# LiMeng95/MultiPoseNet.pytorch

Measured on AMD Instinct MI355X. Metric: images/sec (train fwd+bwd) ResNet101 480x480 bs=32/GPU, higher is better.
Workload: dtype bf16; 1 GPU; R101 full posenet (keypoint+detection) train step: fwd + MSE/focal losses + bwd + Adam, 480x480, 32 images/GPU, bf16 MFMA / fp32 accumulate / fp32 master weights; global_batch=32, parallelism=dp1, loss_log=asynchronous (set_lazy_log), launch=recorded launch list re-issued per step (replay.py), 88 replays, optimizer_update=Adam in one launch after backward

## Files before the change

### include/mpn.h

```cpp
#ifndef MPN_H_
#define MPN_H_
#include <stdint.h>

#ifdef __cplusplus
extern "C" {
#endif

#define MPN_F32 0
#define MPN_BF16 1
#define MPN_F16 2

#define MPN_E_BADARG (-2)
#define MPN_E_UNSUPPORTED (-3)

typedef struct MpnConvParams {
    const void* x;
    const void* w;
    void* y;
    const float* bias;
    const float* scale;
    const void* res;
    const uint8_t* res_mask;
    float* stats;
    int64_t x_sB, x_sH, x_sW;
// ... 81 lines not shown
int mpn_conv_wgrad_reduce(const MpnWgradParams* p, void* stream);
int mpn_conv_wgrad_kernel_id(const MpnWgradParams* p);

int mpn_reduce_partials(const float* ws, int chunks, int64_t n, float* dst, int accumulate, void* stream);

int mpn_cast_f32_to_bf16(const float* src, void* dst, int64_t n, void* stream);
int mpn_cast_f32(const float* src, void* dst, int64_t n, int dtype, void* stream);
int mpn_weight_transpose(const float* w, void* wt, int Cout, int RS, int Cin, int Cout_pad,
                         int dtype, void* stream);
int mpn_weight_transpose_batched(const float* arena, void* dst, const int64_t* table, int nlayers, int64_t nblocks,
                                 int dtype, void* stream);
int mpn_weight_pad_k(const float* w, void* dst, int Cout, int K, int Kpad, int dtype, void* stream);
int mpn_stem_pack_weight(const float* w, void* packed, int Cout, int dtype, void* stream);
int mpn_stem_unpack_wgrad(const float* dpacked, float* dw, int Cout, void* stream);
int mpn_stem_pack_image(const float* img, int64_t sB, int64_t sC, int64_t sH, int64_t sW, void* dst,
                        int B, int H, int W, int dtype, void* stream);

int mpn_bn_finalize_train(const float* stats, int tiles, int C, int64_t count, const float* gamma,
                          const float* beta, float* running_mean, float* running_var, float momentum,
                          float eps, float* mean, float* invstd, float* scale, float* shift, void* stream);
int mpn_bn_finalize_eval(int C, const float* gamma, const float* beta, const float* running_mean,
                         const float* running_var, float eps, float* mean, float* invstd,
                         float* scale, float* shift, void* stream);
int mpn_bn_act_forward(const void* y, const void* res, void* z, const float* scale, const float* shift,
                       int64_t P, int C, int Cs, int relu, int dtype, uint8_t* mask, void* stream);
int mpn_bn_bwd_reduce(const void* dz, const void* z, const void* y, const float* mean, const float* invstd,
                      const float* mask_scale, const float* mask_shift, float* partial, int chunks, int64_t P, int C, int Cs, int relu, int dtype, void* stream);
int mpn_bn_bwd_finalize(const float* partial, int chunks, int C, int64_t count, const float* gamma, const float* mean,
                        const float* invstd, int train, float* dgamma, float* dbeta, float* coef, void* stream);
int mpn_bn_bwd_apply(const void* dz, const void* z, const void* y, const float* k1, const float* k2, const float* k3,
                     const float* mask_scale, const float* mask_shift, void* dy, void* dres, int dres_accumulate, int64_t P, int C, int Cs, int relu, int dtype,
                     const uint8_t* mask, void* stream);
int mpn_bn_bwd_chunks(int64_t P, int Cs, int dtype);

int mpn_maxpool3x3s2_forward(const void* x, void* y, uint8_t* idx, int B, int H, int W, int Cs,
                             int Ho, int Wo, int dtype, void* stream);
int mpn_maxpool3x3s2_backward(const void* dy, const uint8_t* idx, void* dx, int B, int H, int W, int Cs,
                              int Ho, int Wo, int dtype, void* stream);
int mpn_upsample_nearest_backward(const void* dfine, void* dcoarse, int B, int Hf, int Wf, int Hc, int Wc,
                                  int Cs, int accumulate, int dtype, void* stream);
int mpn_upsample_nearest_slice(const void* src, void* dst, int B, int Hs, int Ws, int Cs_src,
                               int Ho, int Wo, int Cs_dst, int c_off, int dtype, void* stream);
int mpn_upsample_nearest_slice_backward(const void* ddst, void* dsrc, int B, int Hs, int Ws, int Cs_src,
                                        int Ho, int Wo, int Cs_dst, int c_off, int dtype, void* stream);
int mpn_export_f32(const void* src, int src_dtype, float* dst, int B, int Hs, int Ws, int Cs, int C,
                   int Ho, int Wo, int64_t dst_sB, int64_t dst_sP, void* stream);
int mpn_import_grad(const float* ddst, int64_t ddst_sB, int64_t ddst_sP, void* dsrc, int dst_dtype,
                    int B, int Hs, int Ws, int Cs, int C, int Ho, int Wo, void* stream);
int mpn_nchw_to_nhwc_f32(const float* src, int64_t sB, int64_t sC, int64_t sH, int64_t sW, float* dst,
                         int B, int C, int H, int W, void* stream);
int mpn_det_pack(const void* src, int src_dtype, float* dst, int B, int64_t HW, int Cs, int C, int64_t dst_sB, void* stream);
int mpn_det_unpack(const float* ddst, void* dsrc, int dst_dtype, int B, int64_t HW, int Cs, int C, int64_t dst_sB, void* stream);
int mpn_relu_forward(const void* x, void* y, int64_t n, int dtype, void* stream);
int mpn_relu_backward(const void* dz, const void* z, void* dx, int64_t n, int accumulate, int dtype, void* stream);
int mpn_add_inplace(void* dst, const void* src, int64_t n, int dtype, void* stream);
int mpn_channel_sum(const void* dy, int dy_dtype, int64_t P, int C, int Cs, float* partial, int chunks, void* stream);
int mpn_channel_sum_chunks(int64_t P, int Cs, int dtype);
int mpn_colsum_rows(const void* dy, int dy_dtype, int64_t P, int C, int Cs, float* db, void* stream);

int mpn_mse_heatmap_forward(const float* const* preds, const int64_t* pred_sP, const float* gt, const float* wgt,
                            int64_t npix, float* partial, int chunks, float* out, void* stream);
int mpn_mse_heatmap_backward(const float* const* preds, float* const* dpreds, const int64_t* pred_sP,
                             const int64_t* dpred_sP, const int32_t* pred_C, const float* gt, const float* wgt,
                             int64_t npix, const float* gscale, void* stream);
int mpn_mse_chunks(int64_t npix);
int mpn_mse_train_blocks(int B, int H, int W);
// ... 104 lines not shown
```

### multiposenet/pytorch_amd/_lib.py

```python
import ctypes
import os
import subprocess

import torch

_HERE = os.path.dirname(os.path.abspath(__file__))
LIB_PATH = os.path.join(_HERE, "libmpn_hip.so")
CSRC = os.path.join(_HERE, "csrc")

F32, BF16, F16 = 0, 1, 2


class MpnError(RuntimeError):
    pass


class ConvParams(ctypes.Structure):
    _fields_ = [
        ("x", ctypes.c_void_p), ("w", ctypes.c_void_p), ("y", ctypes.c_void_p),
        ("bias", ctypes.c_void_p), ("scale", ctypes.c_void_p), ("res", ctypes.c_void_p), ("res_mask", ctypes.c_void_p),
        ("stats", ctypes.c_void_p),
        ("x_sB", ctypes.c_int64), ("x_sH", ctypes.c_int64), ("x_sW", ctypes.c_int64),
        ("y_sB", ctypes.c_int64), ("y_sP", ctypes.c_int64),
        ("res_sB", ctypes.c_int64), ("res_sP", ctypes.c_int64),
# ... 42 lines not shown
    "mpn_resize": (_i, [_vp, _i64, _i64, _i64, _i, _i, _i, _vp, _i, _i, _i, ctypes.c_double, ctypes.c_double, _vp]),
    "mpn_prn_build_maps": (_i, [_vp, _vp, _vp, _vp, _i, _i, _i, ctypes.c_double, _vp, _vp, _vp, _vp, _vp]),
    "mpn_prn_scores": (_i, [_vp, _vp, _i, _i, _i, _i, _vp, _vp, _vp]),
    "mpn_prn_scores_compact": (_i, [_vp, _vp, _i, _i, _i, _i, _i, _vp, _vp, _vp, _vp, _vp, _vp]),
    "mpn_prn_match_host": (_i, [_i, _vp, _vp, _vp, _vp, _vp, _vp, _vp, _i, _vp, _i, _i, _vp, _vp]),
    "mpn_conv_stats_tiles": (_i, [_PC]),
    "mpn_conv_tile_rows": (_i, [_PC]),
    "mpn_conv_shared_tile": (_i, [_PC]),
    "mpn_conv_forward": (_i, [_PC, _vp]),
    "mpn_debug_wgrad_prof": (_i, [_vp]),
    "mpn_debug_igemm_prof": (_i, [_vp]),
    "mpn_conv_wgrad_chunks": (_i, [_PW]),
    "mpn_conv_wgrad_seg_plan": (_i, [_PW]),
    "mpn_conv_wgrad": (_i, [_PW, _vp]),
    "mpn_conv_wgrad_partials": (_i, [_PW, _vp]),
    "mpn_conv_wgrad_reduce": (_i, [_PW, _vp]),
    "mpn_conv_wgrad_kernel_id": (_i, [_PW]),
    "mpn_reduce_partials": (_i, [_vp, _i, _i64, _vp, _i, _vp]),
    "mpn_cast_f32_to_bf16": (_i, [_vp, _vp, _i64, _vp]),
    "mpn_cast_f32": (_i, [_vp, _vp, _i64, _i, _vp]),
    "mpn_weight_transpose": (_i, [_vp, _vp, _i, _i, _i, _i, _i, _vp]),
    "mpn_weight_transpose_batched": (_i, [_vp, _vp, _vp, _i, _i64, _i, _vp]),
    "mpn_weight_pad_k": (_i, [_vp, _vp, _i, _i, _i, _i, _vp]),
    "mpn_stem_pack_weight": (_i, [_vp, _vp, _i, _i, _vp]),
    "mpn_stem_unpack_wgrad": (_i, [_vp, _vp, _i, _vp]),
    "mpn_stem_pack_image": (_i, [_vp, _i64, _i64, _i64, _i64, _vp, _i, _i, _i, _i, _vp]),
    "mpn_bn_finalize_train": (_i, [_vp, _i, _i, _i64, _vp, _vp, _vp, _vp, _f, _f, _vp, _vp, _vp, _vp, _vp]),
    "mpn_bn_finalize_eval": (_i, [_i, _vp, _vp, _vp, _vp, _f, _vp, _vp, _vp, _vp, _vp]),
    "mpn_bn_act_forward": (_i, [_vp, _vp, _vp, _vp, _vp, _i64, _i, _i, _i, _i, _vp, _vp]),
    "mpn_bn_bwd_reduce": (_i, [_vp, _vp, _vp, _vp, _vp, _vp, _vp, _vp, _i, _i64, _i, _i, _i, _i, _vp]),
    "mpn_bn_bwd_finalize": (_i, [_vp, _i, _i, _i64, _vp, _vp, _vp, _i, _vp, _vp, _vp, _vp]),
    "mpn_bn_bwd_apply": (_i, [_vp, _vp, _vp, _vp, _vp, _vp, _vp, _vp, _vp, _vp, _i, _i64, _i, _i, _i, _i, _vp, _vp]),
    "mpn_bn_bwd_chunks": (_i, [_i64, _i, _i]),
    "mpn_maxpool3x3s2_forward": (_i, [_vp, _vp, _vp, _i, _i, _i, _i, _i, _i, _i, _vp]),
    "mpn_maxpool3x3s2_backward": (_i, [_vp, _vp, _vp, _i, _i, _i, _i, _i, _i, _i, _vp]),
    "mpn_upsample_nearest_backward": (_i, [_vp, _vp, _i, _i, _i, _i, _i, _i, _i, _i, _vp]),
    "mpn_upsample_nearest_slice": (_i, [_vp, _vp, _i, _i, _i, _i, _i, _i, _i, _i, _i, _vp]),
    "mpn_upsample_nearest_slice_backward": (_i, [_vp, _vp, _i, _i, _i, _i, _i, _i, _i, _i, _i, _vp]),
    "mpn_export_f32": (_i, [_vp, _i, _vp, _i, _i, _i, _i, _i, _i, _i, _i64, _i64, _vp]),
    "mpn_import_grad": (_i, [_vp, _i64, _i64, _vp, _i, _i, _i, _i, _i, _i, _i, _i, _vp]),
    "mpn_nchw_to_nhwc_f32": (_i, [_vp, _i64, _i64, _i64, _i64, _vp, _i, _i, _i, _i, _vp]),
    "mpn_det_pack": (_i, [_vp, _i, _vp, _i, _i64, _i, _i, _i64, _vp]),
    "mpn_det_unpack": (_i, [_vp, _vp, _i, _i, _i64, _i, _i, _i64, _vp]),
    "mpn_relu_forward": (_i, [_vp, _vp, _i64, _i, _vp]),
    "mpn_relu_backward": (_i, [_vp, _vp, _vp, _i64, _i, _i, _vp]),
    "mpn_add_inplace": (_i, [_vp, _vp, _i64, _i, _vp]),
    "mpn_channel_sum": (_i, [_vp, _i, _i64, _i, _i, _vp, _i, _vp]),
    "mpn_colsum_rows": (_i, [_vp, _i, _i64, _i, _i, _vp, _vp]),
    "mpn_channel_sum_chunks": (_i, [_i64, _i, _i]),
    "mpn_mse_chunks": (_i, [_i64]),
    "mpn_mse_heatmap_forward": (_i, [_vp, _vp, _vp, _vp, _i64, _vp, _i, _vp, _vp]),
    "mpn_mse_heatmap_backward": (_i, [_vp, _vp, _vp, _vp, _vp, _vp, _vp, _i64, _vp, _vp]),
    "mpn_mse_train_blocks": (_i, [_i, _i, _i]),
    "mpn_mse_heatmap_train": (_i, [_vp, _vp, _vp, _i, _vp, _vp, _i64, _i64, _i64, _i, _i, _i, _vp, _vp, _i, _vp, _vp]),
    "mpn_focal_blocks": (_i, [_i]),
    "mpn_focal_forward": (_i, [_vp, _vp, _vp, _vp, _i, _i, _i, _vp, _vp, _vp, _vp]),
    "mpn_focal_backward": (_i, [_vp, _vp, _vp, _vp, _i, _i, _i, _vp, _vp, _vp, _vp, _vp]),
    "mpn_focal_mc_blocks": (_i, [_i]),
    "mpn_focal_forward_mc": (_i, [_vp, _vp, _vp, _vp, _i, _i, _i, _i, _vp, _vp, _vp, _vp, _vp]),
    "mpn_focal_backward_mc": (_i, [_vp, _vp, _vp, _vp, _i, _i, _i, _i, _vp, _vp, _vp, _vp, _vp]),
    "mpn_class_max": (_i, [_vp, _i, _i, _i, _vp, _vp, _vp]),
    "mpn_sigmoid_forward": (_i, [_vp, _vp, _i64, _vp]),
    "mpn_gather_dets": (_i, [_vp, _vp, _i, _vp, _vp, _vp]),
    "mpn_sigmoid_backward": (_i, [_vp, _vp, _vp, _i64, _vp]),
    "mpn_add_softmax_rows": (_i, [_vp, _i64, _vp, _vp, _i, _i, _i, _vp]),
    "mpn_softmax_rows_backward": (_i, [_vp, _vp, _vp, _i64, _vp, _i, _i, _vp]),
# ... 113 lines not shown
```

### multiposenet/pytorch_amd/csrc/bn.hip

```cpp
#include "common.h"
#include <stdlib.h>

namespace {

template <typename T> struct Geo {
    static constexpr int V = Vec16<T>::N;
    int G, GB, lanes, g, pl, c0;
    __device__ __forceinline__ Geo(int Cs) {
        G = Cs / V;
        GB = G < 256 ? G : 256;
        lanes = 256 / GB;
        g = blockIdx.y * GB + (threadIdx.x % GB);
        pl = threadIdx.x / GB;
        c0 = g * V;
    }
};

template <int V>
__device__ __forceinline__ void load_coef(const float* __restrict__ p, int c0, int C, float (&out)[V], float fill) {
#pragma unroll
    for (int k = 0; k < V; k += 4) {
        if (p != nullptr && c0 + k + 3 < C) {
            const float4 t = *reinterpret_cast<const float4*>(p + c0 + k);
            out[k] = t.x; out[k + 1] = t.y; out[k + 2] = t.z; out[k + 3] = t.w;
// ... 87 lines not shown
                                                     const float* __restrict__ scale, const float* __restrict__ shift,
                                                     long P, int C, int Cs, int relu, int iters, unsigned char* __restrict__ mask) {
    constexpr int V = Vec16<T>::N;
    const Geo<T> q(Cs);
    float sc[V], sf[V];
    load_coef<V>(scale, q.c0, C, sc, 0.f);
    load_coef<V>(shift, q.c0, C, sf, 0.f);
    const long p0 = (long)blockIdx.x * q.lanes * iters + q.pl;
    for (int it = 0; it < iters; ++it) {
        const long p = p0 + (long)it * q.lanes;
        if (p >= P) break;
        const long off = p * Cs + q.c0;
        Vec16<T> a; a.load(y + off);
        Vec16<T> r;
        if (res) r.load(res + off);
#pragma unroll
        for (int k = 0; k < V; ++k) {
            float x = a.v[k] * sc[k] + sf[k];
            if (res) x += r.v[k];
            if (relu) x = fmaxf(x, 0.f);
            a.v[k] = (q.c0 + k < C) ? x : 0.f;
        }
        a.store(z + off);
        if (mask) {
            unsigned bits = 0;
#pragma unroll
            for (int k = 0; k < V; ++k) bits |= (Elem<T>::round(a.v[k]) > 0.f ? 1u : 0u) << k;
            mask[p * q.G + q.g] = (unsigned char)bits;
        }
    }
}

template <typename T>
__global__ void __launch_bounds__(256) bn_bwd_reduce_kernel(const T* __restrict__ dz, const T* __restrict__ z, const T* __restrict__ y,
                                                            const float* __restrict__ mean, const float* __restrict__ invstd,
                                                            const float* __restrict__ mscale, const float* __restrict__ mshift,
                                                            float* __restrict__ partial, long P, int C, int Cs, int relu, int chunk_pix) {
    constexpr int V = Vec16<T>::N;
    __shared__ float sh[256][2 * V + 1];
    const Geo<T> q(Cs);
    const long p_begin = (long)blockIdx.x * chunk_pix;
    long p_end = p_begin + chunk_pix; if (p_end > P) p_end = P;
    float s1[V], s2[V], mu[V], is[V], sc[V], sf[V];
    load_coef<V>(mean, q.c0, C, mu, 0.f);
    load_coef<V>(invstd, q.c0, C, is, 0.f);
    const bool remask = relu && z == nullptr;
    if (remask) { load_coef<V>(mscale, q.c0, C, sc, 0.f); load_coef<V>(mshift, q.c0, C, sf, 0.f); }
#pragma unroll
    for (int k = 0; k < V; ++k) { s1[k] = 0.f; s2[k] = 0.f; }
    for (long p = p_begin + q.pl; p < p_end; p += q.lanes) {
        const long off = p * Cs + q.c0;
        Vec16<T> d, o, x;
        d.load(dz + off); x.load(y + off);
        if (relu && !remask) o.load(z + off);
#pragma unroll
        for (int k = 0; k < V; ++k) {
            float gk = d.v[k];
            if (remask) o.v[k] = x.v[k] * sc[k] + sf[k];
            if (relu && !(o.v[k] > 0.f)) gk = 0.f;
            s1[k] += gk;
            s2[k] += gk * ((x.v[k] - mu[k]) * is[k]);
        }
    }
#pragma unroll
    for (int k = 0; k < V; ++k) { sh[threadIdx.x][k] = s1[k]; sh[threadIdx.x][V + k] = s2[k]; }
    __syncthreads();
    if (q.pl == 0) {
        for (int l = 1; l < q.lanes; ++l) {
#pragma unroll
            for (int k = 0; k < V; ++k) {
                s1[k] += sh[threadIdx.x + l * q.GB][k];
                s2[k] += sh[threadIdx.x + l * q.GB][V + k];
            }
        }
#pragma unroll
        for (int k = 0; k < V; ++k) {
            const int c = q.c0 + k;
            if (c < C) *reinterpret_cast<float2*>(partial + ((long)blockIdx.x * C + c) * 2) = make_float2(s1[k], s2[k]);
        }
    }
}

__global__ void bn_bwd_finalize_kernel(const float* __restrict__ partial, int chunks, int C, double count,
                                       const float* __restrict__ gamma, const float* __restrict__ mean, const float* __restrict__ invstd,
                                       int train, float* __restrict__ dgamma, float* __restrict__ dbeta, float* __restrict__ coef) {
    __shared__ double sh[2][4][4];
    const int cl = threadIdx.x & 3, sl = threadIdx.x >> 2;
    const int c = blockIdx.x * 4 + cl;
    double s1 = 0.0, s2 = 0.0;
    const bool fin = sl == 0 && c < C;
    const float is = fin ? invstd[c] : 0.f, gm = (fin && gamma) ? gamma[c] : 1.f, mu = fin ? mean[c] : 0.f;
    const float db0 = (fin && dbeta) ? dbeta[c] : 0.f, dg0 = (fin && dgamma) ? dgamma[c] : 0.f;
    if (c < C) reduce_slices(partial, chunks, C, c, sl, s1, s2);
#pragma unroll
    for (int m = 4; m < 64; m <<= 1) { s1 += __shfl_xor(s1, m); s2 += __shfl_xor(s2, m); }
    const int lane = threadIdx.x & 63, wave = threadIdx.x >> 6;
    if (lane < 4) { sh[0][wave][cl] = s1; sh[1][wave][cl] = s2; }
    __syncthreads();
    if (sl == 0 && c < C) {
        s1 = (sh[0][0][cl] + sh[0][1][cl]) + (sh[0][2][cl] + sh[0][3][cl]);
        s2 = (sh[1][0][cl] + sh[1][1][cl]) + (sh[1][2][cl] + sh[1][3][cl]);
        if (dbeta) dbeta[c] = db0 + (float)s1;
        if (dgamma) dgamma[c] = dg0 + (float)s2;
        if (coef) {
            const float a = (float)(s1 / count), b = (float)(s2 / count);
            coef[c] = gm * is;
            coef[C + c] = train ? -gm * is * is * b : 0.f;
            coef[2 * C + c] = train ? gm * is * (mu * is * b - a) : 0.f;
        }
    }
}

template <typename T>
__global__ void __launch_bounds__(256) bn_bwd_apply_kernel(const T* __restrict__ dz, const T* __restrict__ z, const T* __restrict__ y,
                                                           const float* __restrict__ k1p, const float* __restrict__ k2p,
                                                           const float* __restrict__ k3p, const float* __restrict__ mscale,
                                                           const float* __restrict__ mshift, T* __restrict__ dy, T* __restrict__ dres,
                                                           int dres_acc, long P, int C, int Cs, int relu, int iters,
                                                           const unsigned char* __restrict__ mask) {
    constexpr int V = Vec16<T>::N;
    const Geo<T> q(Cs);
    float k1[V], k2[V], k3[V];
    load_coef<V>(k1p, q.c0, C, k1, 0.f);
    load_coef<V>(k2p, q.c0, C, k2, 0.f);
    load_coef<V>(k3p, q.c0, C, k3, 0.f);
    const bool bits = relu && mask != nullptr;
    const bool remask = relu && !bits && z == nullptr;
    float sc[V], sf[V];
    if (remask) { load_coef<V>(mscale, q.c0, C, sc, 0.f); load_coef<V>(mshift, q.c0, C, sf, 0.f); }
    const bool need_y = ((dy != nullptr) && (k2p != nullptr)) || remask;
    const long p0 = (long)blockIdx.x * q.lanes * iters + q.pl;
    for (int it = 0; it < iters; ++it) {
        const long p = p0 + (long)it * q.lanes;
        if (p >= P) break;
        const long off = p * Cs + q.c0;
        Vec16<T> d, o, x, out, r;
        d.load(dz + off);
        if (need_y) x.load(y + off);
        if (relu && !remask && !bits) o.load(z + off);
        unsigned mb = 0;
        if (bits) mb = mask[p * q.G + q.g];
        if (dres && dres_acc) r.load(dres + off);
#pragma unroll
        for (int k = 0; k < V; ++k) {
            float gk = d.v[k];
            if (remask) o.v[k] = x.v[k] * sc[k] + sf[k];
            if (bits) o.v[k] = ((mb >> k) & 1u) ? 1.f : 0.f;
            if (relu && !(o.v[k] > 0.f)) gk = 0.f;
            const bool live = q.c0 + k < C;
            out.v[k] = live ? (k1[k] * gk + (k2p ? k2[k] * x.v[k] : 0.f) + k3[k]) : 0.f;
            if (dres) r.v[k] = (dres_acc ? r.v[k] : 0.f) + (live ? gk : 0.f);
        }
        if (dy) out.store(dy + off);
        if (dres) r.store(dres + off);
    }
}

inline int geo_lanes(int Cs, int V) { const int G = Cs / V; return 256 / (G < 256 ? G : 256); }
inline int geo_yblocks(int Cs, int V) { const int G = Cs / V; return G <= 256 ? 1 : G / 256; }
inline bool geo_ok(int Cs, int V) { const int G = Cs / V; return Cs % V == 0 && G > 0 && (G & (G - 1)) == 0; }

inline int pick_iters(long P, int lanes) {
    static const long blocks = mpn_tune("MPN_BN_BLOCKS", 8192);
    long it = P / ((long)lanes * blocks);
    if (it < 1) it = 1;
    if (it > 32) it = 32;
    return (int)it;
}
inline int reduce_chunk(long P, int lanes) {
    long c = P / 512;
    const long lo = (long)lanes * 4, hi = 4096;
    if (c < lo) c = lo;
    if (c > hi) c = hi;
    return (int)((c + lanes - 1) / lanes * lanes);
}

}

extern "C" int mpn_bn_finalize_train(const float* stats, int tiles, int C, int64_t count, const float* gamma,
                                     const float* beta, float* running_mean, float* running_var, float momentum,
                                     float eps, float* mean, float* invstd, float* scale, float* shift, void* stream) {
    MPN_CHECK_ARG(stats && tiles > 0 && C > 0 && count > 0 && mean && invstd && scale && shift);
    hipLaunchKernelGGL(bn_finalize_train_kernel, dim3((C + 3) / 4), dim3(256), 0, (hipStream_t)stream, stats, tiles, C,
                       (double)count, gamma, beta, running_mean, running_var, momentum, eps, mean, invstd, scale, shift);
    return mpn_launch_status();
}

extern "C" int mpn_bn_finalize_eval(int C, const float* gamma, const float* beta, const float* running_mean,
                                    const float* running_var, float eps, float* mean, float* invstd,
                                    float* scale, float* shift, void* stream) {
// ... 31 lines not shown
    const int chunk = reduce_chunk(P, geo_lanes(Cs, V));
    MPN_CHECK_ARG(chunks == (int)((P + chunk - 1) / chunk));
    dim3 grid((unsigned)chunks, (unsigned)geo_yblocks(Cs, V));
    MPN_DISPATCH_T(dtype, hipLaunchKernelGGL((bn_bwd_reduce_kernel<T>), grid, dim3(256), 0, (hipStream_t)stream, (const T*)dz, (const T*)z,
                           (const T*)y, mean, invstd, mask_scale, mask_shift, partial, (long)P, C, Cs, relu, chunk));
    return mpn_launch_status();
}

extern "C" int mpn_bn_bwd_finalize(const float* partial, int chunks, int C, int64_t count, const float* gamma, const float* mean,
                                   const float* invstd, int train, float* dgamma, float* dbeta, float* coef, void* stream) {
    MPN_CHECK_ARG(partial && chunks > 0 && C > 0 && count > 0);
    MPN_CHECK_ARG(!coef || (mean && invstd));
    hipLaunchKernelGGL(bn_bwd_finalize_kernel, dim3((C + 3) / 4), dim3(256), 0, (hipStream_t)stream, partial, chunks, C,
                       (double)count, gamma, mean, invstd, train, dgamma, dbeta, coef);
    return mpn_launch_status();
}

extern "C" int mpn_bn_bwd_apply(const void* dz, const void* z, const void* y, const float* k1, const float* k2, const float* k3,
                                const float* mask_scale, const float* mask_shift, void* dy, void* dres, int dres_accumulate, int64_t P, int C, int Cs, int relu, int dtype,
                                const uint8_t* mask, void* stream) {
    MPN_CHECK_ARG(dz && (dy || dres) && P > 0 && C > 0 && Cs >= C);
    MPN_CHECK_ARG(!dy || k1);
    MPN_CHECK_ARG(!(dy && k2) || y);
    MPN_CHECK_ARG(!relu || z || mask || (mask_scale && mask_shift && y));
    const int V = dtype == MPN_F32 ? 4 : 8;
    MPN_CHECK_ARG(geo_ok(Cs, V) && C % 4 == 0);
    const int lanes = geo_lanes(Cs, V), iters = pick_iters(P, lanes);
    dim3 grid((unsigned)((P + (long)lanes * iters - 1) / ((long)lanes * iters)), (unsigned)geo_yblocks(Cs, V));
    MPN_DISPATCH_T(dtype, hipLaunchKernelGGL((bn_bwd_apply_kernel<T>), grid, dim3(256), 0, (hipStream_t)stream, (const T*)dz, (const T*)z,
                           (const T*)y, k1, k2, k3, mask_scale, mask_shift, (T*)dy, (T*)dres, dres_accumulate, (long)P, C, Cs, relu, iters,
                           (const unsigned char*)mask));
    return mpn_launch_status();
}
```

### multiposenet/pytorch_amd/engine.py

```python
import ctypes
import os

import torch

from . import ops
from ._lib import MpnError, call, gpu_op
from .ops import Act, round_up


class Ctx(object):

    def __init__(self, train):
        self.train = train
        self.tape = []
        self.grads = {}
        self.keep = []
        self.out_grads = {}
        self.wt = {}
        self.wt_buf = None
        self.uses = {}
        self.bn_train_ran = False
        self.side_keep = []
        self.side_pending = []
        self.wt_ready = None
# ... 24 lines not shown


def num_classes(cm):
    cout = cm.output.weight.shape[0]
    if cout % 9 != 0 or cout == 0 or getattr(cm, "num_anchors", 9) != 9:
        raise MpnError("classificationModel: the output convolution has %d channels; the detector needs 9 anchors x K classes" % cout)
    return cout // 9


def _geom(layer):
    w = layer.weight
    if w.dim() == 2:
        return w.shape[0], w.shape[1], 1, 1, 1, 0
    return w.shape[0], w.shape[1], w.shape[2], w.shape[3], layer.stride[0], layer.padding[0]


class Engine(object):
    def __init__(self, model):
        self.m = model
        self._drop_calls = 0
        self._side = None
        self._wt_plan_cache = None
        self.overlap_wgrad = os.environ.get("MPN_SIDE_STREAM", "1") != "0"
        self.fork_every = max(1, int(os.environ.get("MPN_SIDE_FORK_EVERY", "1")))
        self.pyramid_towers = os.environ.get("MPN_PYRAMID_TOWERS", "1") != "0"
        self.fuse_bn_stats = os.environ.get("MPN_BN_FUSED_STATS", "1") != "0"
        self.fold_bn = os.environ.get("MPN_FOLD_BN", "1") != "0"
        self.fuse_bn_finalize = os.environ.get("MPN_BN_FUSED_FINALIZE", "1") != "0"
        self.det_pyramid_side = int(os.environ.get("MPN_DET_PYRAMID_SIDE", "2"))
        self.bn_mask_bits = os.environ.get("MPN_BN_MASK_BITS", "1") != "0"
        self.defer_shortcut_grad = os.environ.get("MPN_DEFER_SHORTCUT_GRAD", "1") != "0"
        self.virtual_concat = os.environ.get("MPN_VIRTUAL_CONCAT", "1") != "0"
        self.conv2_classes = os.environ.get("MPN_CONV2_CLASSES", "1") != "0"

    def side_stream(self, device):
        if not self.overlap_wgrad or device.type != "cuda":
            return None
        if self._side is None:
            self._side = torch.cuda.Stream(device=device)
        return self._side

    def _on_side(self, ctx, device, keep, fn, torch_ops=False):
        side = self.side_stream(device)
        if side is None:
            fn()
            return
        ctx.side_keep.append(keep)
        ctx.side_pending.append((fn, torch_ops))
        if len(ctx.side_pending) >= self.fork_every:
            self.flush_side(ctx, device)

    def flush_side(self, ctx, device):
        if not ctx.side_pending:
            return
        side = self.side_stream(device)
        pending, ctx.side_pending = ctx.side_pending, []
        ev = torch.cuda.Event()
        gpu_op(ev.record, torch.cuda.current_stream(device))
        gpu_op(side.wait_event, ev)
        for fn, torch_ops in pending:
            if torch_ops:
                with torch.cuda.stream(side):
                    fn()
                continue
            ops.push_stream(side)
            try:
# ... 645 lines not shown
            img = img.float()
        packed = torch.empty((B, Hp, Wp, 4), dtype=self.cdt, device=img.device)
        call("mpn_stem_pack_image", ops.ptr(img), img.stride(0), img.stride(1), img.stride(2), img.stride(3), ops.ptr(packed),
             B, H, W, ops.dtype_code(self.cdt), ops.stream_ptr())
        xa = Act(packed, 4)
        w = f.conv1.weight
        wp = torch.empty((64, 7, 32), dtype=self.cdt, device=img.device)
        call("mpn_stem_pack_weight", ops.ptr(self.m._arena.data_seg(w)), ops.ptr(wp), 64, ops.dtype_code(self.cdt), ops.stream_ptr())
        Ho, Wo = ops.conv_out_hw(H, W, 7, 7, 2, 3)
        geom = (Hp, Wp, Hp * Wp * 4, Wp * 4, 4)
        bn_train = f.bn1.training
        if self.fold_bn and not ctx.train and not bn_train:
            bst = ops.bn_finalize_eval(f.bn1.weight.data, f.bn1.bias.data, f.bn1.running_mean, f.bn1.running_var, f.bn1.eps)
            z, _ = ops.conv_forward(xa, wp, 64, 7, 1, 2, 0, cin=32, x_geom=geom, out_hw=(Ho, Wo), scale=bst.scale, bias=bst.shift, act=1)
            return self.maxpool(ctx, z)
        y, st = ops.conv_forward(xa, wp, 64, 7, 1, 2, 0, cin=32, x_geom=geom, out_hw=(Ho, Wo), want_stats=bn_train,
                                 bn_fin=self._bn_fin(f.bn1) if bn_train else None)
        if ctx.train and w.requires_grad:
            y.needs_grad = True
            self._note_use(ctx, w)

            def bwd():
                dy = ctx.pop_grad(y)
                if dy is not None:
                    dwp = torch.empty((64, 7, 32), dtype=torch.float32, device=img.device)

                    def stem_wgrad():
                        call("mpn_fill_f32", ops.ptr(dwp), 0.0, dwp.numel(), ops.stream_ptr())
                        ops.conv_wgrad(xa, dy, dwp, 64, 7, 1, 2, 0, cin=32, x_geom=geom)
                        call("mpn_stem_unpack_wgrad", ops.ptr(dwp), ops.ptr(self.m._arena.grad_seg(w)), 64, ops.stream_ptr())
                    self._on_side(ctx, dy.t.device, (xa, dy, dwp), stem_wgrad)
                self._grad_done(ctx, w)
            ctx.tape.append(bwd)
        z = self.bn(ctx, y, st, f.bn1, True)
        return self.maxpool(ctx, z)

    def conv_bn(self, ctx, x, conv, bn, relu, res=None):
        if self.fold_bn and not ctx.train and not bn.training:
            st = ops.bn_finalize_eval(bn.weight.data, bn.bias.data, bn.running_mean, bn.running_var, bn.eps)
            O, I, R, S, stride, pad = _geom(conv)
            act = (3 if res is not None else 1) if relu else 0
            y, _ = ops.conv_forward(x, self.w_fwd(conv), O, R, S, stride, pad, scale=st.scale, bias=st.shift, act=act,
                                    res=res, res_mode=1 if res is not None else 0)
            return y
        y, s = self.conv(ctx, x, conv, stats=bn.training, bn=bn)
        return self.bn(ctx, y, s, bn, relu, res=res)

    def bottleneck(self, ctx, x, blk):
        z1 = self.conv_bn(ctx, x, blk.conv1, blk.bn1, True)
        z2 = self.conv_bn(ctx, z1, blk.conv2, blk.bn2, True)
        sc = self.conv_bn(ctx, x, blk.downsample[0], blk.downsample[1], False) if len(blk.downsample) > 0 else x
        return self.conv_bn(ctx, z2, blk.conv3, blk.bn3, True, res=sc)

    def backbone(self, ctx, img):
        f = self.m.fpn
        c = self.stem(ctx, img)
        feats = []
        for layer in (f.layer1, f.layer2, f.layer3, f.layer4):
            for blk in layer:
                c = self.bottleneck(ctx, c, blk)
            feats.append(c)
        return feats

    def det_pyramid(self, ctx, c3, c4, c5):
        f = self.m.fpn

        def coarse(h):
            h["p6"], _ = self.conv(ctx, c5, f.conv6)
# ... 167 lines not shown
```

### multiposenet/pytorch_amd/ops.py

```python
import ctypes
import os

import torch

from . import _lib
from ._lib import BF16, F16, F32, ConvParams, WgradParams, call


def round_up(v, m):
    return (v + m - 1) // m * m


def dtype_code(dt):
    if dt == torch.float32:
        return F32
    if dt == torch.bfloat16:
        return BF16
    if dt == torch.float16:
        return F16
    raise _lib.MpnError("unsupported dtype %s" % dt)


_STREAM_OVERRIDE = []

# ... 717 lines not shown
                 chunks, P, C, Cs, 1 if relu else 0, dc, stream_ptr())
        coef = torch.empty((3, C), dtype=torch.float32, device=dev) if train else None
        call("mpn_bn_bwd_finalize", ptr(part), chunks, C, P, ptr(gamma), ptr(st.mean), ptr(st.invstd), 1 if train else 0,
             ptr(dgamma), ptr(dbeta), ptr(coef), stream_ptr())
        if train:
            k1, k2, k3 = coef[0], coef[1], coef[2]
    dy = None
    if want_dy or dres is not None:
        if want_dy:
            dy = Act(torch.empty_like(y.t), C)
        bits = z.mask if (relu and not remask) else None
        call("mpn_bn_bwd_apply", ptr(dz.t), ptr(z.t) if (relu and not remask and bits is None) else None, ptr(y.t), ptr(k1), ptr(k2), ptr(k3),
             ptr(st.scale) if remask else None, ptr(st.shift) if remask else None,
             ptr(dy.t) if dy is not None else None, ptr(dres.t) if dres is not None else None,
             1 if dres_acc else 0, P, C, Cs, 1 if relu else 0, dc, ptr(bits), stream_ptr())
    return dy


def maxpool_forward(x, needs_grad=False):
    Ho, Wo = (x.H + 2 - 3) // 2 + 1, (x.W + 2 - 3) // 2 + 1
    y = Act(torch.empty((x.B, Ho, Wo, x.Cs), dtype=x.t.dtype, device=x.t.device), x.C, needs_grad)
    idx = torch.empty((x.B, Ho, Wo, x.Cs), dtype=torch.uint8, device=x.t.device) if needs_grad else None
    call("mpn_maxpool3x3s2_forward", ptr(x.t), ptr(y.t), ptr(idx), x.B, x.H, x.W, x.Cs, Ho, Wo, dtype_code(x.t.dtype), stream_ptr())
    return y, idx


def maxpool_backward(dy, idx, x_like):
    dx = Act(torch.empty_like(x_like.t), x_like.C)
    call("mpn_maxpool3x3s2_backward", ptr(dy.t), ptr(idx), ptr(dx.t), x_like.B, x_like.H, x_like.W, x_like.Cs, dy.H, dy.W,
         dtype_code(dy.t.dtype), stream_ptr())
    return dx


def upsample_backward(dfine, dcoarse, accumulate):
    call("mpn_upsample_nearest_backward", ptr(dfine.t), ptr(dcoarse.t), dfine.B, dfine.H, dfine.W, dcoarse.H, dcoarse.W,
         dfine.Cs, 1 if accumulate else 0, dtype_code(dfine.t.dtype), stream_ptr())


def upsample_slice(src, dst, c_off):
    call("mpn_upsample_nearest_slice", ptr(src.t), ptr(dst.t), src.B, src.H, src.W, src.Cs, dst.H, dst.W, dst.Cs, c_off,
         dtype_code(src.t.dtype), stream_ptr())


def upsample_slice_backward(ddst, dsrc, c_off):
    call("mpn_upsample_nearest_slice_backward", ptr(ddst.t), ptr(dsrc.t), dsrc.B, dsrc.H, dsrc.W, dsrc.Cs, ddst.H, ddst.W,
         ddst.Cs, c_off, dtype_code(dsrc.t.dtype), stream_ptr())


def export_f32(src, C, Ho, Wo):
    out = torch.empty((src.B, Ho, Wo, C), dtype=torch.float32, device=src.t.device)
    call("mpn_export_f32", ptr(src.t), dtype_code(src.t.dtype), ptr(out), src.B, src.H, src.W, src.Cs, C, Ho, Wo,
         Ho * Wo * C, C, stream_ptr())
    return out.permute(0, 3, 1, 2)


def import_grad(g_nchw, like, dtype):
    B, C, Ho, Wo = g_nchw.shape
    g = g_nchw.permute(0, 2, 3, 1)
    if g.stride(3) != 1 or g.stride(1) != Wo * g.stride(2):
        g = g.contiguous()
    d = Act(torch.empty((like.B, like.H, like.W, like.Cs), dtype=dtype, device=like.t.device), like.C)
    call("mpn_import_grad", ptr(g), g.stride(0), g.stride(2), ptr(d.t), dtype_code(dtype), like.B, like.H, like.W, like.Cs,
         like.C, Ho, Wo, stream_ptr())
    return d


# ... 163 lines not shown
```

### multiposenet/pytorch_amd/replay.py

```python
import itertools
import math
import os
from collections import OrderedDict

import ctypes

import torch

from . import _lib, ops
from .engine import Ctx
from .network import losses

_epoch = itertools.count(1 << 20)


class _Entry(object):
    __slots__ = ("tape", "pool", "img", "gts", "logv", "names", "keep", "sig", "loss")


class ReplayedTrainStep(object):
    def __init__(self, model, optimizer, eager_steps=1, fused_mse=None, max_entries=None, anno_bucket=8, max_grad_norm=None):
        self.model = model
        self.opt = optimizer
        self.max_grad_norm = None if max_grad_norm is None or math.isinf(max_grad_norm) else float(max_grad_norm)
# ... 77 lines not shown
        return self.bucket_mode == "1" or self.model._reducer is not None

    def _local_schedule(self):
        from .ddp import GradReducer
        ar = self.model._arena
        sc = getattr(self, "_local", None)
        if sc is None or sc.arena is not ar:
            sc = self._local = GradReducer(ar, local=True, bucket_mb=float(os.environ.get("MPN_BUCKET_MB", "32")))
        return sc

    def _ones(self, dev):
        t = getattr(self, "_ones_t", None)
        if t is None or t.device != dev:
            t = self._ones_t = torch.ones(2, dtype=torch.float32, device=dev)
        return t

    @staticmethod
    def _log_names(want_kp, want_det, clip=False):
        names = []
        if want_kp:
            kn = losses.build_names()
            names += [(kn[j * 2], j) for j in range(5)] + [("max_ht", 6), ("min_ht", 7)]
        if want_det:
            names += [("total_loss", 8), ("classification_loss", 9), ("regression_loss", 10)]
        if clip:
            names.append(("max_grad", 12))
        return names

    def _state_sig(self):
        m = self.model
        ar = m._arena
        return (id(ar), id(ar.grad_flat), tuple(p.requires_grad for p in ar.params), tuple(b.training for b in m._bns),
                m.compute_dtype, id(m._reducer), m._engine.overlap_wgrad, m._engine.fork_every, id(self.opt._m), self.bucketed_update,
                m._engine.conv2_classes, m._engine.virtual_concat, self._clip_sig())

    def _clip_sig(self):
        if self.max_grad_norm is None:
            return None
        return tuple(p.grad is not None for p in self.model._arena.params)

    def __call__(self, inputs, gts):
        (img, subnet), = inputs
        gts = list(gts)
        if gts[0] != subnet:
            raise ValueError("inputs and gts name different subnets (%r vs %r)" % (subnet, gts[0]))
        tensors = gts[1:]
        if subnet not in ("keypoint_subnet", "detection_subnet", "train_both"):
            if self.max_grad_norm is not None:
                raise ValueError("recorded train step: %r is not recorded and train_step does not clip; clip it on the eager path "
                                 "(training.trainer._Stepper does)" % (subnet,))
            from .training.batch_processor import train_step
            return train_step(self.model, self.opt, inputs, gts)
        ops.check_device(img)
        img = self._as_f32(img, "image batch")
        tensors = [self._as_f32(g, "target %d" % i) for i, g in enumerate(tensors)]
        if subnet in ("detection_subnet", "train_both") and self.anno_bucket > 1:
            ai = 2 if subnet == "train_both" else 0
            if ai < len(tensors) and tensors[ai].dim() == 3:
                tensors[ai] = self._bucket_annotations(tensors[ai])
        key = (subnet, tuple(img.shape), img.dtype, tuple((tuple(t.shape), t.dtype) for t in tensors))
        ent = self._entries.get(key)
        if ent is not None and ent.sig != self._state_sig():
            ent = None
            self._drop(key)
        if ent is not None:
            self._entries.move_to_end(key)
        if ent is None:
# ... 99 lines not shown
```

Before: 894.1 images/sec.

## Fuse stem BN+ReLU with 3x3 maxpool forward and backward

Adds a kernel that applies the stem's BN scale/shift and ReLU while computing the 3x3 stride-2 maxpool and argmax indices, so the full-resolution activated tensor is never written. The backward pass feeds pooled gradients and indices straight into the BN backward reduce and apply kernels, which rebuild the unpooled gradient on the fly. This removes the maxpool backward kernel and the full-resolution z and dz round trips. In exchange each pixel does extra index gathers, and the work is duplicated across the reduce and apply passes. The path is on by default and can be disabled with an environment flag.

```diff
diff --git a/include/mpn.h b/include/mpn.h
--- a/include/mpn.h
+++ b/include/mpn.h
@@ -137,6 +137,14 @@
                      const float* mask_scale, const float* mask_shift, void* dy, void* dres, int dres_accumulate, int64_t P, int C, int Cs, int relu, int dtype,
                      const uint8_t* mask, void* stream);
 int mpn_bn_bwd_chunks(int64_t P, int Cs, int dtype);
+int mpn_bn_act_maxpool_forward(const void* y, void* out, uint8_t* idx, const float* scale, const float* shift,
+                               int B, int H, int W, int Ho, int Wo, int C, int Cs, int dtype, void* stream);
+int mpn_bn_bwd_reduce_pooled(const void* dp, const uint8_t* idx, const void* y, const float* mean, const float* invstd,
+                             const float* mask_scale, const float* mask_shift, float* partial, int chunks,
+                             int B, int H, int W, int Ho, int Wo, int C, int Cs, int dtype, void* stream);
+int mpn_bn_bwd_apply_pooled(const void* dp, const uint8_t* idx, const void* y, const float* k1, const float* k2, const float* k3,
+                            const float* mask_scale, const float* mask_shift, void* dy,
+                            int B, int H, int W, int Ho, int Wo, int C, int Cs, int dtype, void* stream);
 
 int mpn_maxpool3x3s2_forward(const void* x, void* y, uint8_t* idx, int B, int H, int W, int Cs,
                              int Ho, int Wo, int dtype, void* stream);
diff --git a/multiposenet/pytorch_amd/_lib.py b/multiposenet/pytorch_amd/_lib.py
--- a/multiposenet/pytorch_amd/_lib.py
+++ b/multiposenet/pytorch_amd/_lib.py
@@ -98,6 +98,9 @@
     "mpn_bn_bwd_finalize": (_i, [_vp, _i, _i, _i64, _vp, _vp, _vp, _i, _vp, _vp, _vp, _vp]),
     "mpn_bn_bwd_apply": (_i, [_vp, _vp, _vp, _vp, _vp, _vp, _vp, _vp, _vp, _vp, _i, _i64, _i, _i, _i, _i, _vp, _vp]),
     "mpn_bn_bwd_chunks": (_i, [_i64, _i, _i]),
+    "mpn_bn_act_maxpool_forward": (_i, [_vp] * 5 + [_i] * 8 + [_vp]),
+    "mpn_bn_bwd_reduce_pooled": (_i, [_vp] * 8 + [_i] * 9 + [_vp]),
+    "mpn_bn_bwd_apply_pooled": (_i, [_vp] * 9 + [_i] * 8 + [_vp]),
     "mpn_maxpool3x3s2_forward": (_i, [_vp, _vp, _vp, _i, _i, _i, _i, _i, _i, _i, _vp]),
     "mpn_maxpool3x3s2_backward": (_i, [_vp, _vp, _vp, _i, _i, _i, _i, _i, _i, _i, _vp]),
     "mpn_upsample_nearest_backward": (_i, [_vp, _vp, _i, _i, _i, _i, _i, _i, _i, _i, _vp]),
diff --git a/multiposenet/pytorch_amd/csrc/bn.hip b/multiposenet/pytorch_amd/csrc/bn.hip
--- a/multiposenet/pytorch_amd/csrc/bn.hip
+++ b/multiposenet/pytorch_amd/csrc/bn.hip
@@ -143,14 +143,120 @@
 }
 
 template <typename T>
-__global__ void __launch_bounds__(256) bn_bwd_reduce_kernel(const T* __restrict__ dz, const T* __restrict__ z, const T* __restrict__ y,
-                                                            const float* __restrict__ mean, const float* __restrict__ invstd,
-                                                            const float* __restrict__ mscale, const float* __restrict__ mshift,
-                                                            float* __restrict__ partial, long P, int C, int Cs, int relu, int chunk_pix) {
+__global__ void __launch_bounds__(256) bn_act_maxpool_kernel(const T* __restrict__ y, T* __restrict__ out, unsigned char* __restrict__ idx,
+                                                             const float* __restrict__ scale, const float* __restrict__ shift,
+                                                             int B, int H, int W, int Ho, int Wo, int C, int Cs, int iters) {
     constexpr int V = Vec16<T>::N;
-    __shared__ float sh[256][2 * V + 1];
     const Geo<T> q(Cs);
-    const long p_begin = (long)blockIdx.x * chunk_pix;
+    float sc[V], sf[V];
+    load_coef<V>(scale, q.c0, C, sc, 0.f);
+    load_coef<V>(shift, q.c0, C, sf, 0.f);
+    const int Po = B * Ho * Wo;
+    const int p0 = xcd_remap(blockIdx.x, gridDim.x) * q.lanes * iters + q.pl;
+    for (int it = 0; it < iters; ++it) {
+        const int p = p0 + it * q.lanes;
+        if (p >= Po) break;
+        const int wo = p % Wo, t = p / Wo;
+        const int ho = t % Ho, b = t / Ho;
+        float best[V];
+        unsigned bi[V];
+#pragma unroll
+        for (int k = 0; k < V; ++k) { best[k] = -INFINITY; bi[k] = 0; }
+        const bool vr[3] = {ho > 0, true, ho * 2 + 1 < H}, vs[3] = {wo > 0, true, wo * 2 + 1 < W};
+        uint4 raw[9];
+#pragma unroll
+        for (int r = 0; r < 3; ++r) {
+            const long rowoff = ((long)b * H + (vr[r] ? ho * 2 - 1 + r : ho * 2)) * W;
+#pragma unroll
+            for (int s = 0; s < 3; ++s)
+                raw[r * 3 + s] = *reinterpret_cast<const uint4*>(y + (rowoff + (vs[s] ? wo * 2 - 1 + s : wo * 2)) * Cs + q.c0);
+        }
+#pragma unroll
+        for (int t = 0; t < 9; ++t) {
+            __builtin_amdgcn_sched_barrier(0);
+            const bool valid = vr[t / 3] && vs[t % 3];
+            Vec16<T> a; a.load(reinterpret_cast<const T*>(&raw[t]));
+#pragma unroll
+            for (int k = 0; k < V; ++k) {
+                const float x = fmaxf(a.v[k] * sc[k] + sf[k], 0.f);
+                const float z = Elem<T>::round((q.c0 + k < C) ? x : 0.f);
+                if (valid && z > best[k]) { best[k] = z; bi[k] = t; }
+            }
+        }
+        __builtin_amdgcn_sched_barrier(0);
+        const long off = (long)p * Cs + q.c0;
+        Vec16<T> o;
+#pragma unroll
+        for (int k = 0; k < V; ++k) o.v[k] = best[k];
+        o.store(out + off);
+        if (idx) {
+            unsigned lo = 0, hi = 0;
+#pragma unroll
+            for (int k = 0; k < V; ++k) { if (k < 4) lo |= bi[k] << (8 * k); else hi |= bi[k] << (8 * (k - 4)); }
+            if (V == 8) *reinterpret_cast<uint2*>(idx + off) = make_uint2(lo, hi);
+            else *reinterpret_cast<unsigned*>(idx + off) = lo;
+        }
+    }
+}
+
+template <typename T> struct DzLoad {
+    static constexpr bool kRemap = false;
+    const T* dz;
+    __device__ __forceinline__ void get(Vec16<T>& d, long p, long off) const { d.load(dz + off); }
+};
+template <typename T> struct DzPooled {
+    static constexpr bool kRemap = true;
+    const T* dp;
+    const unsigned char* idx;
+    int H, W, Ho, Wo, Cs, c0;
+    __device__ __forceinline__ void get(Vec16<T>& d, long p, long) const {
+        constexpr int V = Vec16<T>::N;
+        const int pi = (int)p;
+        const int w = pi % W, t = pi / W;
+        const int h = t % H, b = t / H;
+        const int ho0 = h >> 1, wo0 = w >> 1;
+        const bool vh = (h & 1) && ho0 + 1 < Ho, vw = (w & 1) && wo0 + 1 < Wo;
+        const unsigned r0 = ((h & 1) + 1) * 3, s0 = (w & 1) + 1;
+        const long o00 = (((long)b * Ho + ho0) * Wo + wo0) * Cs + c0;
+        const long o01 = o00 + (vw ? Cs : 0);
+        const long row = vh ? (long)Wo * Cs : 0;
+        Vec16<T> v[4];
+        unsigned lo[4], hi[4];
+        load(v[0], lo[0], hi[0], o00);
+        load(v[1], lo[1], hi[1], o01);
+        load(v[2], lo[2], hi[2], o00 + row);
+        load(v[3], lo[3], hi[3], o01 + row);
+        const unsigned tap[4] = {r0 + s0, vw ? r0 : 0xffu, vh ? s0 : 0xffu, (vh && vw) ? 0u : 0xffu};
+        float acc[V];
+#pragma unroll
+        for (int k = 0; k < V; ++k) acc[k] = 0.f;
+#pragma unroll
+        for (int i = 0; i < 4; ++i) {
+#pragma unroll
+            for (int k = 0; k < V; ++k)
+                if ((((k < 4 ? lo[i] : hi[i]) >> (8 * (k & 3))) & 0xffu) == tap[i]) acc[k] += v[i].v[k];
+        }
+#pragma unroll
+        for (int k = 0; k < V; ++k) d.v[k] = Elem<T>::round(acc[k]);
+    }
+    __device__ __forceinline__ void load(Vec16<T>& v, unsigned& lo, unsigned& hi, long o) const {
+        v.load(dp + o);
+        hi = 0;
+        if (Vec16<T>::N == 8) { const uint2 m = *reinterpret_cast<const uint2*>(idx + o); lo = m.x; hi = m.y; }
+        else lo = *reinterpret_cast<const unsigned*>(idx + o);
+    }
+};
+
+template <typename T, typename Src>
+__device__ __forceinline__ void bn_bwd_reduce_body(const Src src, const T* __restrict__ z, const T* __restrict__ y,
+                                                   const float* __restrict__ mean, const float* __restrict__ invstd,
+                                                   const float* __restrict__ mscale, const float* __restrict__ mshift,
+                                                   float* __restrict__ partial, long P, int C, int Cs, int relu, int chunk_pix,
+                                                   float (*sh)[2 * Vec16<T>::N + 1]) {
+    constexpr int V = Vec16<T>::N;
+    const Geo<T> q(Cs);
+    const int chunk = Src::kRemap ? xcd_remap(blockIdx.x, gridDim.x) : blockIdx.x;
+    const long p_begin = (long)chunk * chunk_pix;
     long p_end = p_begin + chunk_pix; if (p_end > P) p_end = P;
     float s1[V], s2[V], mu[V], is[V], sc[V], sf[V];
     load_coef<V>(mean, q.c0, C, mu, 0.f);
@@ -162,7 +268,8 @@
     for (long p = p_begin + q.pl; p < p_end; p += q.lanes) {
         const long off = p * Cs + q.c0;
         Vec16<T> d, o, x;
-        d.load(dz + off); x.load(y + off);
+        x.load(y + off);
+        src.get(d, p, off);
         if (relu && !remask) o.load(z + off);
 #pragma unroll
         for (int k = 0; k < V; ++k) {
@@ -187,9 +294,30 @@
 #pragma unroll
         for (int k = 0; k < V; ++k) {
             const int c = q.c0 + k;
-            if (c < C) *reinterpret_cast<float2*>(partial + ((long)blockIdx.x * C + c) * 2) = make_float2(s1[k], s2[k]);
-        }
-    }
+            if (c < C) *reinterpret_cast<float2*>(partial + ((long)chunk * C + c) * 2) = make_float2(s1[k], s2[k]);
+        }
+    }
+}
+
+template <typename T>
+__global__ void __launch_bounds__(256) bn_bwd_reduce_kernel(const T* __restrict__ dz, const T* __restrict__ z, const T* __restrict__ y,
+                                                            const float* __restrict__ mean, const float* __restrict__ invstd,
+                                                            const float* __restrict__ mscale, const float* __restrict__ mshift,
+                                                            float* __restrict__ partial, long P, int C, int Cs, int relu, int chunk_pix) {
+    __shared__ float sh[256][2 * Vec16<T>::N + 1];
+    bn_bwd_reduce_body<T>(DzLoad<T>{dz}, z, y, mean, invstd, mscale, mshift, partial, P, C, Cs, relu, chunk_pix, sh);
+}
+
+template <typename T>
+__global__ void __launch_bounds__(256) bn_bwd_reduce_pooled_kernel(const T* __restrict__ dp, const unsigned char* __restrict__ idx,
+                                                                   int H, int W, int Ho, int Wo, const T* __restrict__ y,
+                                                                   const float* __restrict__ mean, const float* __restrict__ invstd,
+                                                                   const float* __restrict__ mscale, const float* __restrict__ mshift,
+                                                                   float* __restrict__ partial, long P, int C, int Cs, int relu, int chunk_pix) {
+    __shared__ float sh[256][2 * Vec16<T>::N + 1];
+    const Geo<T> q(Cs);
+    bn_bwd_reduce_body<T>(DzPooled<T>{dp, idx, H, W, Ho, Wo, Cs, q.c0}, (const T*)nullptr, y, mean, invstd, mscale, mshift, partial,
+                          P, C, Cs, relu, chunk_pix, sh);
 }
 
 __global__ void bn_bwd_finalize_kernel(const float* __restrict__ partial, int chunks, int C, double count,
@@ -222,13 +350,13 @@
     }
 }
 
-template <typename T>
-__global__ void __launch_bounds__(256) bn_bwd_apply_kernel(const T* __restrict__ dz, const T* __restrict__ z, const T* __restrict__ y,
-                                                           const float* __restrict__ k1p, const float* __restrict__ k2p,
-                                                           const float* __restrict__ k3p, const float* __restrict__ mscale,
-                                                           const float* __restrict__ mshift, T* __restrict__ dy, T* __restrict__ dres,
-                                                           int dres_acc, long P, int C, int Cs, int relu, int iters,
-                                                           const unsigned char* __restrict__ mask) {
+template <typename T, typename Src>
+__device__ __forceinline__ void bn_bwd_apply_body(const Src src, const T* __restrict__ z, const T* __restrict__ y,
+                                                  const float* __restrict__ k1p, const float* __restrict__ k2p,
+                                                  const float* __restrict__ k3p, const float* __restrict__ mscale,
+                                                  const float* __restrict__ mshift, T* __restrict__ dy, T* __restrict__ dres,
+                                                  int dres_acc, long P, int C, int Cs, int relu, int iters,
+                                                  const unsigned char* __restrict__ mask) {
     constexpr int V = Vec16<T>::N;
     const Geo<T> q(Cs);
     float k1[V], k2[V], k3[V];
@@ -240,14 +368,14 @@
     float sc[V], sf[V];
     if (remask) { load_coef<V>(mscale, q.c0, C, sc, 0.f); load_coef<V>(mshift, q.c0, C, sf, 0.f); }
     const bool need_y = ((dy != nullptr) && (k2p != nullptr)) || remask;
-    const long p0 = (long)blockIdx.x * q.lanes * iters + q.pl;
+    const long p0 = (long)(Src::kRemap ? xcd_remap(blockIdx.x, gridDim.x) : blockIdx.x) * q.lanes * iters + q.pl;
     for (int it = 0; it < iters; ++it) {
         const long p = p0 + (long)it * q.lanes;
         if (p >= P) break;
         const long off = p * Cs + q.c0;
         Vec16<T> d, o, x, out, r;
-        d.load(dz + off);
         if (need_y) x.load(y + off);
+        src.get(d, p, off);
         if (relu && !remask && !bits) o.load(z + off);
         unsigned mb = 0;
         if (bits) mb = mask[p * q.G + q.g];
@@ -267,6 +395,28 @@
     }
 }
 
+template <typename T>
+__global__ void __launch_bounds__(256) bn_bwd_apply_kernel(const T* __restrict__ dz, const T* __restrict__ z, const T* __restrict__ y,
+                                                           const float* __restrict__ k1p, const float* __restrict__ k2p,
+                                                           const float* __restrict__ k3p, const float* __restrict__ mscale,
+                                                           const float* __restrict__ mshift, T* __restrict__ dy, T* __restrict__ dres,
+                                                           int dres_acc, long P, int C, int Cs, int relu, int iters,
+                                                           const unsigned char* __restrict__ mask) {
+    bn_bwd_apply_body<T>(DzLoad<T>{dz}, z, y, k1p, k2p, k3p, mscale, mshift, dy, dres, dres_acc, P, C, Cs, relu, iters, mask);
+}
+
+template <typename T>
+__global__ void __launch_bounds__(256) bn_bwd_apply_pooled_kernel(const T* __restrict__ dp, const unsigned char* __restrict__ idx,
+                                                                  int H, int W, int Ho, int Wo, const T* __restrict__ y,
+                                                                  const float* __restrict__ k1p, const float* __restrict__ k2p,
+                                                                  const float* __restrict__ k3p, const float* __restrict__ mscale,
+                                                                  const float* __restrict__ mshift, T* __restrict__ dy,
+                                                                  long P, int C, int Cs, int relu, int iters) {
+    const Geo<T> q(Cs);
+    bn_bwd_apply_body<T>(DzPooled<T>{dp, idx, H, W, Ho, Wo, Cs, q.c0}, (const T*)nullptr, y, k1p, k2p, k3p, mscale, mshift, dy, (T*)nullptr, 0,
+                         P, C, Cs, relu, iters, (const unsigned char*)nullptr);
+}
+
 inline int geo_lanes(int Cs, int V) { const int G = Cs / V; return 256 / (G < 256 ? G : 256); }
 inline int geo_yblocks(int Cs, int V) { const int G = Cs / V; return G <= 256 ? 1 : G / 256; }
 inline bool geo_ok(int Cs, int V) { const int G = Cs / V; return Cs % V == 0 && G > 0 && (G & (G - 1)) == 0; }
@@ -364,3 +514,55 @@
                            (const unsigned char*)mask));
     return mpn_launch_status();
 }
+
+namespace {
+inline bool pool_geo_ok(int B, int H, int W, int Ho, int Wo) {
+    return B > 0 && H > 0 && W > 0 && Ho == (H + 2 - 3) / 2 + 1 && Wo == (W + 2 - 3) / 2 + 1 && (long)B * H * W < (1L << 31) / 2;
+}
+}
+
+extern "C" int mpn_bn_act_maxpool_forward(const void* y, void* out, uint8_t* idx, const float* scale, const float* shift,
+                                          int B, int H, int W, int Ho, int Wo, int C, int Cs, int dtype, void* stream) {
+    MPN_CHECK_ARG(y && out && scale && shift && C > 0 && Cs >= C && mpn_dtype_ok(dtype) && pool_geo_ok(B, H, W, Ho, Wo));
+    const int V = dtype == MPN_F32 ? 4 : 8;
+    MPN_CHECK_ARG(geo_ok(Cs, V) && C % 4 == 0);
+    const long Po = (long)B * Ho * Wo;
+    const int lanes = geo_lanes(Cs, V), iters = pick_iters(Po, lanes);
+    dim3 grid((unsigned)((Po + (long)lanes * iters - 1) / ((long)lanes * iters)), (unsigned)geo_yblocks(Cs, V));
+    MPN_DISPATCH_T(dtype, hipLaunchKernelGGL((bn_act_maxpool_kernel<T>), grid, dim3(256), 0, (hipStream_t)stream, (const T*)y, (T*)out,
+                           (unsigned char*)idx, scale, shift, B, H, W, Ho, Wo, C, Cs, iters));
+    return mpn_launch_status();
+}
+
+extern "C" int mpn_bn_bwd_reduce_pooled(const void* dp, const uint8_t* idx, const void* y, const float* mean, const float* invstd,
+                                        const float* mask_scale, const float* mask_shift, float* partial, int chunks,
+                                        int B, int H, int W, int Ho, int Wo, int C, int Cs, int dtype, void* stream) {
+    MPN_CHECK_ARG(dp && idx && y && mean && invstd && partial && C > 0 && Cs >= C && mpn_dtype_ok(dtype) && pool_geo_ok(B, H, W, Ho, Wo));
+    MPN_CHECK_ARG(mask_scale && mask_shift);
+    const int V = dtype == MPN_F32 ? 4 : 8;
+    MPN_CHECK_ARG(geo_ok(Cs, V) && C % 4 == 0);
+    const long P = (long)B * H * W;
+    const int chunk = reduce_chunk(P, geo_lanes(Cs, V));
+    MPN_CHECK_ARG(chunks == (int)((P + chunk - 1) / chunk));
+    dim3 grid((unsigned)chunks, (unsigned)geo_yblocks(Cs, V));
+    MPN_DISPATCH_T(dtype, hipLaunchKernelGGL((bn_bwd_reduce_pooled_kernel<T>), grid, dim3(256), 0, (hipStream_t)stream, (const T*)dp,
+                           (const unsigned char*)idx, H, W, Ho, Wo, (const T*)y, mean, invstd, mask_scale, mask_shift, partial, P, C, Cs,
+                           1, chunk));
+    return mpn_launch_status();
+}
+
+extern "C" int mpn_bn_bwd_apply_pooled(const void* dp, const uint8_t* idx, const void* y, const float* k1, const float* k2, const float* k3,
+                                       const float* mask_scale, const float* mask_shift, void* dy,
+                                       int B, int H, int W, int Ho, int Wo, int C, int Cs, int dtype, void* stream) {
+    MPN_CHECK_ARG(dp && idx && y && dy && k1 && C > 0 && Cs >= C && mpn_dtype_ok(dtype) && pool_geo_ok(B, H, W, Ho, Wo));
+    MPN_CHECK_ARG(mask_scale && mask_shift);
+    const int V = dtype == MPN_F32 ? 4 : 8;
+    MPN_CHECK_ARG(geo_ok(Cs, V) && C % 4 == 0);
+    const long P = (long)B * H * W;
+    const int lanes = geo_lanes(Cs, V), iters = pick_iters(P, lanes);
+    dim3 grid((unsigned)((P + (long)lanes * iters - 1) / ((long)lanes * iters)), (unsigned)geo_yblocks(Cs, V));
+    MPN_DISPATCH_T(dtype, hipLaunchKernelGGL((bn_bwd_apply_pooled_kernel<T>), grid, dim3(256), 0, (hipStream_t)stream, (const T*)dp,
+                           (const unsigned char*)idx, H, W, Ho, Wo, (const T*)y, k1, k2, k3, mask_scale, mask_shift, (T*)dy, P, C, Cs,
+                           1, iters));
+    return mpn_launch_status();
+}
diff --git a/multiposenet/pytorch_amd/engine.py b/multiposenet/pytorch_amd/engine.py
--- a/multiposenet/pytorch_amd/engine.py
+++ b/multiposenet/pytorch_amd/engine.py
@@ -80,6 +80,7 @@
         self.defer_shortcut_grad = os.environ.get("MPN_DEFER_SHORTCUT_GRAD", "1") != "0"
         self.virtual_concat = os.environ.get("MPN_VIRTUAL_CONCAT", "1") != "0"
         self.conv2_classes = os.environ.get("MPN_CONV2_CLASSES", "1") != "0"
+        self.stem_pool_fused = os.environ.get("MPN_STEM_POOL_FUSED", "1") != "0"
 
     def side_stream(self, device):
         if not self.overlap_wgrad or device.type != "cuda":
@@ -791,8 +792,39 @@
                     self._on_side(ctx, dy.t.device, (xa, dy, dwp), stem_wgrad)
                 self._grad_done(ctx, w)
             ctx.tape.append(bwd)
+        if bn_train and self.stem_pool_fused:
+            return self._stem_bn_pool(ctx, y, st, f.bn1)
         z = self.bn(ctx, y, st, f.bn1, True)
         return self.maxpool(ctx, z)
+
+    def _stem_bn_pool(self, ctx, y, stats, layer):
+        if isinstance(stats, ops.BNState):
+            st = stats
+        else:
+            st = ops.bn_finalize_train(stats, y.P, layer.weight.data, layer.bias.data, layer.running_mean, layer.running_var,
+                                       layer.momentum if layer.momentum is not None else 0.1, layer.eps)
+        ctx.bn_train_ran = True
+        wg, bg = layer.weight.requires_grad, layer.bias.requires_grad
+        need = bool(ctx.train and (y.needs_grad or wg or bg))
+        p, idx = ops.bn_act_maxpool(y, st, needs_grad=need)
+        if need:
+            self._note_use(ctx, layer.weight)
+            self._note_use(ctx, layer.bias)
+            ar = self.m._arena
+
+            def bwd():
+                dp = ctx.pop_grad(p)
+                if dp is not None:
+                    dy = ops.bn_backward_pooled(dp, idx, y, st, layer.weight.data, dgamma=ar.grad_seg(layer.weight) if wg else None,
+                                                dbeta=ar.grad_seg(layer.bias) if bg else None, want_dy=y.needs_grad)
+                if wg:
+                    self._grad_done(ctx, layer.weight)
+                if bg:
+                    self._grad_done(ctx, layer.bias)
+                if dp is not None and y.needs_grad:
+                    ctx.set_grad(y, dy)
+            ctx.tape.append(bwd)
+        return p
 
     def conv_bn(self, ctx, x, conv, bn, relu, res=None):
         if self.fold_bn and not ctx.train and not bn.training:
diff --git a/multiposenet/pytorch_amd/ops.py b/multiposenet/pytorch_amd/ops.py
--- a/multiposenet/pytorch_amd/ops.py
+++ b/multiposenet/pytorch_amd/ops.py
@@ -773,6 +773,34 @@
     return dx
 
 
+def bn_act_maxpool(y, st, needs_grad=False):
+    Ho, Wo = (y.H + 2 - 3) // 2 + 1, (y.W + 2 - 3) // 2 + 1
+    p = Act(torch.empty((y.B, Ho, Wo, y.Cs), dtype=y.t.dtype, device=y.t.device), y.C, needs_grad)
+    idx = torch.empty((y.B, Ho, Wo, y.Cs), dtype=torch.uint8, device=y.t.device) if needs_grad else None
+    call("mpn_bn_act_maxpool_forward", ptr(y.t), ptr(p.t), ptr(idx), ptr(st.scale), ptr(st.shift), y.B, y.H, y.W, Ho, Wo, y.C, y.Cs,
+         dtype_code(y.t.dtype), stream_ptr())
+    return p, idx
+
+
+def bn_backward_pooled(dp, idx, y, st, gamma, dgamma=None, dbeta=None, want_dy=True):
+    dev = y.t.device
+    C, Cs, dc = y.C, y.Cs, dtype_code(y.t.dtype)
+    geo = (y.B, y.H, y.W, dp.H, dp.W, C, Cs, dc)
+    chunks = call("mpn_bn_bwd_chunks", y.P, Cs, dc)
+    part = workspace(chunks * C * 2 * 4, dev, slot=3)
+    call("mpn_bn_bwd_reduce_pooled", ptr(dp.t), ptr(idx), ptr(y.t), ptr(st.mean), ptr(st.invstd), ptr(st.scale), ptr(st.shift), ptr(part),
+         chunks, *geo, stream_ptr())
+    coef = torch.empty((3, C), dtype=torch.float32, device=dev)
+    call("mpn_bn_bwd_finalize", ptr(part), chunks, C, y.P, ptr(gamma), ptr(st.mean), ptr(st.invstd), 1, ptr(dgamma), ptr(dbeta), ptr(coef),
+         stream_ptr())
+    if not want_dy:
+        return None
+    dy = Act(torch.empty_like(y.t), C)
+    call("mpn_bn_bwd_apply_pooled", ptr(dp.t), ptr(idx), ptr(y.t), ptr(coef[0]), ptr(coef[1]), ptr(coef[2]), ptr(st.scale), ptr(st.shift),
+         ptr(dy.t), *geo, stream_ptr())
+    return dy
+
+
 def upsample_backward(dfine, dcoarse, accumulate):
     call("mpn_upsample_nearest_backward", ptr(dfine.t), ptr(dcoarse.t), dfine.B, dfine.H, dfine.W, dcoarse.H, dcoarse.W,
          dfine.Cs, 1 if accumulate else 0, dtype_code(dfine.t.dtype), stream_ptr())
diff --git a/multiposenet/pytorch_amd/replay.py b/multiposenet/pytorch_amd/replay.py
--- a/multiposenet/pytorch_amd/replay.py
+++ b/multiposenet/pytorch_amd/replay.py
@@ -133,7 +133,7 @@
         ar = m._arena
         return (id(ar), id(ar.grad_flat), tuple(p.requires_grad for p in ar.params), tuple(b.training for b in m._bns),
                 m.compute_dtype, id(m._reducer), m._engine.overlap_wgrad, m._engine.fork_every, id(self.opt._m), self.bucketed_update,
-                m._engine.conv2_classes, m._engine.virtual_concat, self._clip_sig())
+                m._engine.conv2_classes, m._engine.virtual_concat, m._engine.stem_pool_fused, self._clip_sig())
 
     def _clip_sig(self):
         if self.max_grad_norm is None:
```

Result: no change. 898.0 images/sec, median of 6 (+0.4%).
